# MiniMax-AI/VTP

Measured on NVIDIA H100. Metric: images/sec (256x256 encode+decode+3-loss step), higher is better.
Workload: dtype bf16

## Files before the change

vtp_b200/csrc/gemm.cu:

```cuda
#include <stdlib.h>

#include "host.h"
#include "ptx.cuh"

namespace vtp {

static constexpr int BM = 128;
static constexpr int BK = 64;
static constexpr int A_BYTES = BM * BK * 2;
static constexpr int NUM_THREADS = 512;
static constexpr int NUM_MMA_WARPS = 8;

struct GemmDev {
    int M, N, K;
    int a_mn, b_mn;
    int num_m_blocks, num_n_blocks, num_k_blocks, kb_per_split, num_splits;
    void* out;
    int ldo, out_dtype;
    const float* bias;
    int act, round_bf16;
    const void* resid;
    int ldr, resid_dtype;
    int accumulate;
    int rr_group, rr_skip;
    const __nv_bfloat16* rope_sin;
    const __nv_bfloat16* rope_cos;
    int rope_tokens, rope_prefix, rope_cols;
    int ps_r, ps_gh, ps_gw, ps_cout;
    __nv_bfloat16* out2;
    int ldo2;
    int conv_C, conv_H, conv_W, conv_TW, conv_TH, conv_tiles_h, conv_tiles_w, conv_B;
    const __nv_bfloat16* mask_pos;
    int ldm;
};
// ... 267 lines not shown
            store_half<PS>(p, stg, lane, grow0, orow8, ocol0, h, ncols, Nout, 0, has_resid);
            __syncwarp();
        }
    }
}


__device__ __forceinline__ int acc_key(int r) { return ((r & 3) << 1) | ((r >> 2) & 1); }

__device__ __forceinline__ void acc_ld32(const float* arow, int col0, int key, uint32_t (&r)[32]) {
#pragma unroll
    for (int i = 0; i < 8; ++i) {
        const float4 v = *reinterpret_cast<const float4*>(arow + col0 + 4 * (i ^ key));
        r[4 * i] = __float_as_uint(v.x), r[4 * i + 1] = __float_as_uint(v.y), r[4 * i + 2] = __float_as_uint(v.z),
        r[4 * i + 3] = __float_as_uint(v.w);
    }
}

struct AccHandoff {
    uint64_t* full;
    uint64_t* empty;
    uint32_t phase;
    __device__ __forceinline__ void wait_full() const { mbar_wait(full, phase); }
    __device__ __forceinline__ void release(int lane) const {
        __syncwarp();
        if (lane == 0) mbar_arrive(empty);
    }
};

struct TileIter {
    int n, m, ks;
    int dn, dm, dks;
    int nn, nm;
    __device__ __forceinline__ TileIter(int t0, int stride, int num_n, int num_m) : nn(num_n), nm(num_m) {
        n = t0 % num_n;
        const int r = t0 / num_n;
        m = r % num_m, ks = r / num_m;
        dn = stride % num_n;
        const int rs = stride / num_n;
        dm = rs % num_m, dks = rs / num_m;
    }
    __device__ __forceinline__ void next() {
        n += dn, m += dm, ks += dks;
        if (n >= nn) n -= nn, ++m;
        if (m >= nm) m -= nm, ++ks;
    }
};

template <int BN, int FAST>
__device__ __forceinline__ void fast_swiglu_tile(const GemmDev& p, const CUtensorMap* tmO, const CUtensorMap* tmO2, uint8_t* stg,
                                                 uint8_t* stg2, float* bias_s, int lane, int q, const AccHandoff& ah,
                                                 const float* arow, int key, int m_blk, int n0) {
    static_assert(BN == 128, "one packed chunk pair = one 64-column hidden line per tile row");
    constexpr bool PRE = FAST == 6;
    const int m0 = m_blk * BM;
    const int N = p.N;
    ah.wait_full();
    {
#pragma unroll
        for (int j = 0; j < 2; ++j) {
            const int col0 = n0 + j * 64;
            const bool valid = col0 < N;
            uint32_t r0[32], r1[32];
            if (valid) {
                acc_ld32(arow, j * 64, key, r0);
                acc_ld32(arow, j * 64 + 32, key, r1);
            }
            if (j == 1) ah.release(lane);
            bias_s[lane] = (p.bias && col0 + lane < N) ? __ldg(p.bias + col0 + lane) : 0.f;
            bias_s[32 + lane] = (p.bias && col0 + 32 + lane < N) ? __ldg(p.bias + col0 + 32 + lane) : 0.f;
            if (lane == 0) bulk_wait_read0();
            __syncwarp();
            uint32_t hw[16];
            uint32_t xs[32];
// ... 26 lines not shown
#pragma unroll
            for (int c = 0; c < 4; ++c)
                *reinterpret_cast<uint4*>(stg2 + stgb_off(lane, 4 * j + c)) = make_uint4(hw[4 * c], hw[4 * c + 1], hw[4 * c + 2], hw[4 * c + 3]);
            if (PRE && valid) {
                fence_proxy_async_smem();
                __syncwarp();
                if (lane == 0) {
                    tma_store_2d(tmO2, stg, col0, m0 + q * 32);
                    bulk_commit();
                }
            }
        }
        fence_proxy_async_smem();
        __syncwarp();
        if (lane == 0) {
            tma_store_2d(tmO, stg2, n0 >> 1, m0 + q * 32);
            bulk_commit();
        }
    }
}

template <int BN, int ACT, int FAST>
__device__ __forceinline__ void fast_epilogue_tile(const GemmDev& p, const CUtensorMap* tmO, uint8_t* stg, float* bias_s,
                                                   int lane, int q, const AccHandoff& ah, const float* arow, int key,
                                                   int m_blk, int n0) {
    constexpr bool OF32 = FAST == 3 || FAST == 4;
    constexpr bool MASK = FAST == 5;
    constexpr bool RES = FAST == 2 || FAST == 4 || MASK;
    const int m0 = m_blk * BM;
    constexpr int CW = OF32 ? 32 : 64;
    constexpr int TCH = BN / CW;
    constexpr int PW = OF32 ? 4 : 8;
    const int N = p.N;
    long row = (long)m0 + q * 32 + lane;
    bool row_ok = row < p.M;
    int ctx = 0, cty = 0, cb = 0;
    if (p.conv_C) {
        ctx = m_blk % p.conv_tiles_w, cty = (m_blk / p.conv_tiles_w) % p.conv_tiles_h;
        cb = m_blk / (p.conv_tiles_w * p.conv_tiles_h);
        const int r = q * 32 + lane;
        const int h = cty * p.conv_TH + r / p.conv_TW, w = ctx * p.conv_TW + r % p.conv_TW;
        row = ((long)cb * p.conv_H + h) * p.conv_W + w;
        row_ok = h < p.conv_H && cb < p.conv_B;
    }
    const char* rrow = !RES ? nullptr
                       : MASK ? reinterpret_cast<const char*>(p.mask_pos) + row * (long)p.ldm * 2
                              : reinterpret_cast<const char*>(p.resid) + row * (long)p.ldr * (OF32 ? 4 : 2);

    float b0n = 0.f, b1n = 0.f;
    uint4 rr[8];
    auto load_bias = [&](int col0) {
        if (p.bias) {
            b0n = (col0 + lane < N) ? __ldg(p.bias + col0 + lane) : 0.f;
            if (!OF32) b1n = (col0 + 32 + lane < N) ? __ldg(p.bias + col0 + 32 + lane) : 0.f;
        }
    };
    auto load_resid = [&](int col0) {
#pragma unroll
        for (int i = 0; i < 8; ++i) {
            const int col = col0 + PW * i;
            rr[i] = (row_ok && col + PW <= N) ? *reinterpret_cast<const uint4*>(rrow + (long)col * (OF32 ? 4 : 2))
                                              : make_uint4(0, 0, 0, 0);
        }
    };
    load_bias(n0);
    if (RES) {
        load_resid(n0);
#pragma unroll
        for (int j = 1; j < TCH; ++j) {
            const int col = n0 + j * CW;
            if (row_ok && col < N) asm volatile("prefetch.global.L2 [%0];" ::"l"(rrow + (long)col * (OF32 ? 4 : 2)));
        }
    }
    ah.wait_full();
#pragma unroll
    for (int c = 0; c < TCH; ++c) {
        const int col0 = n0 + c * CW;
        if (col0 >= N) break;
        const bool last = (c == TCH - 1) || (col0 + CW >= N);
        const float b0 = b0n, b1 = b1n;
        if (!last) load_bias(col0 + CW);
        uint32_t r0[32], r1[32];
        acc_ld32(arow, c * CW, key, r0);
        if (!OF32) acc_ld32(arow, c * CW + 32, key, r1);
        if (last) ah.release(lane);
        bias_s[lane] = b0;
        if (!OF32) bias_s[32 + lane] = b1;
        if (lane == 0) bulk_wait_read0();
        __syncwarp();
        {
#pragma unroll
            for (int i = 0; i < 8; ++i) {
                if constexpr (OF32) {
                    const float4 b = *reinterpret_cast<const float4*>(bias_s + 4 * i);
                    float4 v = make_float4(__uint_as_float(r0[4 * i]) + b.x, __uint_as_float(r0[4 * i + 1]) + b.y,
                                           __uint_as_float(r0[4 * i + 2]) + b.z, __uint_as_float(r0[4 * i + 3]) + b.w);
                    if (p.round_bf16) v.x = bf16_round(v.x), v.y = bf16_round(v.y), v.z = bf16_round(v.z), v.w = bf16_round(v.w);
                    if (ACT == VTP_ACT_RELU) v.x = fmaxf(v.x, 0.f), v.y = fmaxf(v.y, 0.f), v.z = fmaxf(v.z, 0.f), v.w = fmaxf(v.w, 0.f);
                    if (RES)
                        v.x += __uint_as_float(rr[i].x), v.y += __uint_as_float(rr[i].y), v.z += __uint_as_float(rr[i].z),
                            v.w += __uint_as_float(rr[i].w);
                    *reinterpret_cast<float4*>(stg + stgb_off(lane, i)) = v;
                } else {
                    const float4 ba = *reinterpret_cast<const float4*>(bias_s + 8 * i);
                    const float4 bb = *reinterpret_cast<const float4*>(bias_s + 8 * i + 4);
                    const uint32_t* r = i < 4 ? r0 + 8 * i : r1 + 8 * (i - 4);
                    float v[8] = {__uint_as_float(r[0]) + ba.x, __uint_as_float(r[1]) + ba.y, __uint_as_float(r[2]) + ba.z,
                                  __uint_as_float(r[3]) + ba.w, __uint_as_float(r[4]) + bb.x, __uint_as_float(r[5]) + bb.y,
// ... 8 lines not shown
                    if (MASK) {
                        auto keep = [](uint32_t x, uint32_t mm) {
                            const uint32_t lo = ((mm & 0x7FFFu) != 0u && (mm & 0x8000u) == 0u) ? 0x0000FFFFu : 0u;
                            const uint32_t hi = ((mm & 0x7FFF0000u) != 0u && (mm & 0x80000000u) == 0u) ? 0xFFFF0000u : 0u;
                            return x & (lo | hi);
                        };
                        w.x = keep(w.x, rr[i].x), w.y = keep(w.y, rr[i].y), w.z = keep(w.z, rr[i].z), w.w = keep(w.w, rr[i].w);
                    } else if (RES) {
                        w.x = add_bf16x2(w.x, rr[i].x), w.y = add_bf16x2(w.y, rr[i].y), w.z = add_bf16x2(w.z, rr[i].z),
                        w.w = add_bf16x2(w.w, rr[i].w);
                    }
                    *reinterpret_cast<uint4*>(stg + stgb_off(lane, i)) = w;
                }
            }
            if (RES && !last) load_resid(col0 + CW);
            fence_proxy_async_smem();
            __syncwarp();
            if (lane == 0) {
                if (p.conv_C) tma_store_4d(tmO, stg, col0, ctx * p.conv_TW, cty * p.conv_TH + q * (32 / p.conv_TW), cb);
                else tma_store_2d(tmO, stg, col0, m0 + q * 32);
                bulk_commit();
            }
        }
    }
}

template <int BN, int STAGES, int TA, int TB>
__device__ __forceinline__ void gemm_mainloop(float (&acc)[BN / 2], uint8_t* ring, uint64_t* full_bar, uint64_t* empty_bar,
                                              int& s, uint32_t& ph, int nkb, int wg, int lane) {
    constexpr int STAGE_BYTES = A_BYTES + BN * BK * 2;
    int prev = -1;
    for (int kb = 0; kb < nkb; ++kb) {
        mbar_wait(&full_bar[s], ph);
        const uint32_t a_base = smem_u32(ring + s * STAGE_BYTES) + wg * 8192;
        const uint32_t b_base = smem_u32(ring + s * STAGE_BYTES + A_BYTES);
        wgmma_fence();
#pragma unroll
        for (int j = 0; j < BK / 16; ++j) {
            const uint64_t ad = TA ? wgmma_desc_sw128(a_base + j * 2048, 8192, 1024) : wgmma_desc_sw128(a_base + j * 32, 0, 1024);
            const uint64_t bd = TB ? wgmma_desc_sw128(b_base + j * 2048, 8192, 1024) : wgmma_desc_sw128(b_base + j * 32, 0, 1024);
            const uint32_t sc = (kb > 0 || j > 0) ? 1u : 0u;
            if constexpr (BN == 128) wgmma_m64n128_ss<TA, TB>(acc, ad, bd, sc);
            else wgmma_m64n64_ss<TA, TB>(acc, ad, bd, sc);
        }
        wgmma_commit();
        wgmma_wait<1>();
        fence_regs(acc);
        if (prev >= 0 && lane == 0) mbar_arrive(&empty_bar[prev]);
        prev = s;
        if (++s == STAGES) s = 0, ph ^= 1;
    }
    wgmma_wait<0>();
    fence_regs(acc);
    if (prev >= 0 && lane == 0) mbar_arrive(&empty_bar[prev]);
}

template <int BN, int STAGES, int ACT, bool PS, int FAST>
__global__ void __launch_bounds__(NUM_THREADS, 1)
gemm_kernel(const __grid_constant__ CUtensorMap tmA, const __grid_constant__ CUtensorMap tmB,
            const __grid_constant__ CUtensorMap tmO, const __grid_constant__ CUtensorMap tmO2, const GemmDev p) {
    static_assert(BN == 64 || BN == 128, "tile width");
    constexpr int B_BYTES = BN * BK * 2;
    constexpr int STAGE_BYTES = A_BYTES + B_BYTES;
    extern __shared__ __align__(1024) uint8_t smem_raw[];
    uint8_t* smem = reinterpret_cast<uint8_t*>((reinterpret_cast<uintptr_t>(smem_raw) + 1023) & ~uintptr_t(1023));
    constexpr int STG_BYTES = NUM_EPI_WARPS * STG_FLOATS * 4 * (FAST == 6 ? 2 : 1);
    uint8_t* ring = smem;
    float* acc_s = reinterpret_cast<float*>(ring + STAGES * STAGE_BYTES);
    float* stg_base = acc_s + BM * BN;
    float* bias_base = reinterpret_cast<float*>(reinterpret_cast<uint8_t*>(stg_base) + STG_BYTES);
    uint64_t* full_bar = reinterpret_cast<uint64_t*>(reinterpret_cast<uint8_t*>(bias_base) + (FAST ? NUM_EPI_WARPS * 256 : 0));
    uint64_t* empty_bar = full_bar + STAGES;
    uint64_t* acc_full = empty_bar + STAGES;
    uint64_t* acc_empty = acc_full + 1;

    const int warp = threadIdx.x >> 5;
    const int lane = threadIdx.x & 31;
    const int work_id = blockIdx.x;
    const int work_stride = gridDim.x;

    if (warp == 0 && lane == 0) {
        tma_prefetch_desc(&tmA);
        tma_prefetch_desc(&tmB);
        if (FAST) tma_prefetch_desc(&tmO);
        if (FAST == 6) tma_prefetch_desc(&tmO2);
        for (int s = 0; s < STAGES; ++s) mbar_init(&full_bar[s], 1), mbar_init(&empty_bar[s], NUM_MMA_WARPS);
        mbar_init(acc_full, NUM_MMA_WARPS);
        mbar_init(acc_empty, NUM_EPI_WARPS);
        fence_barrier_init();
    }
    __syncthreads();

    const int num_tiles = p.num_m_blocks * p.num_n_blocks * p.num_splits;
    if (warp < 4) {
        setmaxnreg_dec<40>();
        if (warp == 0 && lane == 0) {
            int s = 0;
            uint32_t ph = 0;
            TileIter ti(work_id, work_stride, p.num_n_blocks, p.num_m_blocks);
            for (int t = work_id; t < num_tiles; t += work_stride, ti.next()) {
                const int n_blk = ti.n, m_blk = ti.m, ks = ti.ks;
                const int kb0 = ks * p.kb_per_split;
                const int kb1 = min(kb0 + p.kb_per_split, p.num_k_blocks);
                const int m0 = m_blk * BM, n0 = n_blk * BN;
                int cv_x0 = 0, cv_y0 = 0, cv_b = 0, cv_c = 0, cv_dx = -1, cv_dy = -1;
                if (p.conv_C) {
                    cv_x0 = (m_blk % p.conv_tiles_w) * p.conv_TW;
                    cv_y0 = ((m_blk / p.conv_tiles_w) % p.conv_tiles_h) * p.conv_TH;
                    cv_b = m_blk / (p.conv_tiles_w * p.conv_tiles_h);
                    if (kb0 != 0) {
                        const int cpk = p.conv_C >> 6, tap = kb0 / cpk;
                        cv_c = (kb0 % cpk) << 6, cv_dx = tap % 3 - 1, cv_dy = tap / 3 - 1;
                    }
                }
                for (int kb = kb0; kb < kb1; ++kb) {
                    mbar_wait(&empty_bar[s], ph ^ 1);
                    uint8_t* sa = ring + s * STAGE_BYTES;
                    uint8_t* sb = sa + A_BYTES;
// ... 3 lines not shown
                        tma_load_4d(sa, &tmA, &full_bar[s], cv_c, cv_x0 + cv_dx, cv_y0 + cv_dy, cv_b);
                        cv_c += 64;
                        if (cv_c == p.conv_C) {
                            cv_c = 0;
                            if (++cv_dx == 2) cv_dx = -1, ++cv_dy;
                        }
                    } else if (!p.a_mn) {
                        tma_load_2d(sa, &tmA, &full_bar[s], k0, m0);
                    } else {
                        tma_load_2d(sa, &tmA, &full_bar[s], m0, k0);
                        tma_load_2d(sa + 8192, &tmA, &full_bar[s], m0 + 64, k0);
                    }
                    if (!p.b_mn) {
                        tma_load_2d(sb, &tmB, &full_bar[s], k0, n0);
                    } else {
#pragma unroll
                        for (int i = 0; i < BN / 64; ++i) tma_load_2d(sb + i * 8192, &tmB, &full_bar[s], n0 + 64 * i, k0);
                    }
                    if (++s == STAGES) s = 0, ph ^= 1;
                }
            }
        }
    } else if (warp < 4 + NUM_MMA_WARPS) {
        setmaxnreg_inc<144>();
        const int wg = (warp >> 2) - 1;
        const int tw = threadIdx.x & 127;
        int s = 0;
        uint32_t ph = 0, acc_ph = 0;
        TileIter ti(work_id, work_stride, p.num_n_blocks, p.num_m_blocks);
        for (int t = work_id; t < num_tiles; t += work_stride, ti.next()) {
            const int kb0 = ti.ks * p.kb_per_split;
            const int nkb = min(kb0 + p.kb_per_split, p.num_k_blocks) - kb0;
            float acc[BN / 2];
            if (p.a_mn) {
                if (p.b_mn) gemm_mainloop<BN, STAGES, 1, 1>(acc, ring, full_bar, empty_bar, s, ph, nkb, wg, lane);
                else gemm_mainloop<BN, STAGES, 1, 0>(acc, ring, full_bar, empty_bar, s, ph, nkb, wg, lane);
            } else {
                if (p.b_mn) gemm_mainloop<BN, STAGES, 0, 1>(acc, ring, full_bar, empty_bar, s, ph, nkb, wg, lane);
                else gemm_mainloop<BN, STAGES, 0, 0>(acc, ring, full_bar, empty_bar, s, ph, nkb, wg, lane);
            }
            mbar_wait(acc_empty, acc_ph ^ 1);
            {
                const int r0 = 64 * wg + 16 * (tw >> 5) + ((tw & 31) >> 2), c0 = 2 * (tw & 3);
                const int key = acc_key(r0);
#pragma unroll
                for (int j = 0; j < BN / 8; ++j) {
                    const int off = 4 * ((2 * j + (c0 >> 2)) ^ key) + (c0 & 3);
                    *reinterpret_cast<float2*>(acc_s + r0 * BN + off) = make_float2(acc[4 * j], acc[4 * j + 1]);
                    *reinterpret_cast<float2*>(acc_s + (r0 + 8) * BN + off) = make_float2(acc[4 * j + 2], acc[4 * j + 3]);
                }
            }
            __syncwarp();
            if (lane == 0) mbar_arrive(acc_full);
            acc_ph ^= 1;
        }
    } else {
        setmaxnreg_inc<184>();
        const int q = warp & 3;
        float* stg = stg_base + q * STG_FLOATS;
        const bool has_resid = p.resid != nullptr;
        const float* arow = acc_s + (q * 32 + lane) * BN;
        const int key = acc_key(lane);
        AccHandoff ah{acc_full, acc_empty, 0};
        TileIter ti(work_id, work_stride, p.num_n_blocks, p.num_m_blocks);
        for (int t = work_id; t < num_tiles; t += work_stride, ti.next(), ah.phase ^= 1) {
            const int m_blk = ti.m, n0 = ti.n * BN;
            const int m0 = m_blk * BM;
            const int grow0 = m0 + q * 32;
            if constexpr (FAST == 6 || FAST == 7) {
                uint8_t* st1 = reinterpret_cast<uint8_t*>(stg);
                uint8_t* st2 = FAST == 6 ? reinterpret_cast<uint8_t*>(stg_base) + (NUM_EPI_WARPS + q) * STG_FLOATS * 4 : st1;
                fast_swiglu_tile<BN, FAST>(p, &tmO, &tmO2, st1, st2, bias_base + q * 64, lane, q, ah, arow, key, m_blk, n0);
                continue;
            }
            if constexpr (FAST != 0) {
                fast_epilogue_tile<BN, ACT, FAST>(p, &tmO, reinterpret_cast<uint8_t*>(stg), bias_base + q * 64, lane, q, ah,
                                                  arow, key, m_blk, n0);
                continue;
            }
            constexpr bool sw = ACT == VTP_ACT_SWIGLU8;
            long orow8[8];
#pragma unroll
            for (int it = 0; it < 8; ++it) orow8[it] = out_row(p, grow0 + 4 * it + (lane >> 3));
            uint32_t hold[16];
            ah.wait_full();
#pragma unroll 1
            for (int u = 0; u < BN / 64; ++u) {
                const int col0 = n0 + u * 64;
                if (col0 >= p.N) break;
                if (has_resid)
                    prefetch_resid_l2(p, lane, orow8, sw ? col0 >> 1 : col0, sw ? 32 : 64, sw ? p.N >> 1 : p.N);
                uint32_t r0[32], r1[32];
                acc_ld32(arow, u * 64, key, r0);
                acc_ld32(arow, u * 64 + 32, key, r1);
                if (u == BN / 64 - 1 || col0 + 64 >= p.N) ah.release(lane);
                float v[64];
#pragma unroll
                for (int i = 0; i < 32; ++i) v[i] = __uint_as_float(r0[i]), v[32 + i] = __uint_as_float(r1[i]);
                epilogue_unit<ACT, PS>(p, stg, lane, v, grow0, orow8, col0, has_resid, sw ? (u & 1) : 0, hold);
            }
        }
        if (FAST && lane == 0) bulk_wait0();
    }
}

template <int BN, int STAGES, int ACT, bool PS, int FAST = 0>
static int launch_gemm(const CUtensorMap& tmA, const CUtensorMap& tmB, const GemmDev& p, cudaStream_t stream,
                       const CUtensorMap* tmO = nullptr, const CUtensorMap* tmO2 = nullptr) {
    constexpr int smem_bytes = 1024 + STAGES * (A_BYTES + BN * BK * 2) + BM * BN * 4 +
                               NUM_EPI_WARPS * STG_FLOATS * 4 * (FAST == 6 ? 2 : 1) + (FAST ? NUM_EPI_WARPS * 256 : 0) +
                               (2 * STAGES + 2) * 8;
    static_assert(smem_bytes <= 232448, "shared memory budget (227 KB per block)");
    static bool configured = false;
    if (!configured) {
        VTP_CUDA(cudaFuncSetAttribute(gemm_kernel<BN, STAGES, ACT, PS, FAST>, cudaFuncAttributeMaxDynamicSharedMemorySize,
                                      smem_bytes));
        configured = true;
    }
    const int work = p.num_m_blocks * p.num_n_blocks * p.num_splits;
    const int grid = work < num_sms() ? work : num_sms();
    gemm_kernel<BN, STAGES, ACT, PS, FAST><<<grid, NUM_THREADS, smem_bytes, stream>>>(tmA, tmB, tmO ? *tmO : tmA,
                                                                                     tmO2 ? *tmO2 : tmA, p);
    VTP_LAUNCH_CHECK();
    return VTP_OK;
}

}

using namespace vtp;

extern "C" int vtp_gemm_bf16(const vtp_gemm_args* a, vtp_stream_t stream_) {
    cudaStream_t stream = reinterpret_cast<cudaStream_t>(stream_);
    VTP_CHECK_ARG(a != nullptr, "gemm: null args");
    VTP_CHECK_ARG(a->M > 0 && a->N > 0 && a->K > 0, "gemm: bad shape M=%d N=%d K=%d", a->M, a->N, a->K);
    VTP_CHECK_ARG(a->A && a->B && a->out, "gemm: null pointer");
    VTP_CHECK_ARG(a->lda % 8 == 0 && a->ldb % 8 == 0, "gemm: lda/ldb must be multiples of 8 (16B TMA strides)");
    VTP_CHECK_ARG((reinterpret_cast<uintptr_t>(a->A) & 15) == 0 && (reinterpret_cast<uintptr_t>(a->B) & 15) == 0,
                  "gemm: A/B must be 16B aligned");
    VTP_CHECK_ARG((reinterpret_cast<uintptr_t>(a->out) & 15) == 0, "gemm: out must be 16B aligned");
    VTP_CHECK_ARG(a->N % 8 == 0, "gemm: N must be a multiple of 8");
    VTP_CHECK_ARG(a->out_dtype == VTP_F32 || a->out_dtype == VTP_BF16, "gemm: bad out dtype");
    VTP_CHECK_ARG(a->ldo % (a->out_dtype == VTP_F32 ? 4 : 8) == 0 || a->ps_r > 0, "gemm: ldo alignment");
    int split_k = a->split_k < 1 ? 1 : a->split_k;
    const bool auto_split = a->split_k < 0 && a->accumulate && a->out_dtype == VTP_F32 && a->act == VTP_ACT_NONE && !a->bias;
    VTP_CHECK_ARG(split_k == 1 || (a->accumulate && a->out_dtype == VTP_F32 && a->act == VTP_ACT_NONE && !a->bias),
                  "gemm: split_k needs accumulate=1, fp32 out, no bias/activation");
    VTP_CHECK_ARG(!a->accumulate || a->out_dtype == VTP_F32, "gemm: accumulate needs fp32 out");
    if (a->act == VTP_ACT_ROPE)
        VTP_CHECK_ARG(a->rope_sin && a->rope_cos && a->rope_tokens > 0 && a->rope_cols % 64 == 0, "gemm: bad rope args");
    if (a->act == VTP_ACT_SWIGLU8) VTP_CHECK_ARG(a->N % 16 == 0, "gemm: swiglu needs N %% 16 == 0");
    if (a->ps_r > 0)
        VTP_CHECK_ARG(a->ps_r % 4 == 0 && a->M % (a->ps_gh * a->ps_gw) == 0 && a->N == a->ps_cout * a->ps_r * a->ps_r,
                      "gemm: bad pixel-shuffle args");
    if (a->resid) VTP_CHECK_ARG(a->ldr % (a->resid_dtype == VTP_F32 ? 4 : 8) == 0, "gemm: ldr alignment");
    if (a->out2) VTP_CHECK_ARG(a->ldo2 % 8 == 0, "gemm: ldo2 alignment");

    const bool conv = a->conv_C > 0;
    if (conv) {
        VTP_CHECK_ARG(a->conv_C % 64 == 0 && a->conv_H > 0 && a->conv_W % 4 == 0 && !a->a_mn_major && a->K == 9 * a->conv_C &&
                          a->M % (a->conv_H * a->conv_W) == 0 && a->rr_group == 0 && a->ps_r == 0,
                      "gemm(conv): need C %% 64 == 0, W %% 4 == 0, K == 9*C, M == B*H*W");
    }
    if (a->mask_pos) VTP_CHECK_ARG(a->out_dtype == VTP_BF16 && a->ldm % 8 == 0, "gemm: mask_pos needs bf16 out");
    int BN = a->N <= 64 ? 64 : 128;
    const bool allow_fast = getenv("VTP_GEMM_NO_FAST") == nullptr;
    const bool fast_conv = conv && a->out_dtype == VTP_BF16 && !a->resid && getenv("VTP_GEMM_CONV_NO_FAST") == nullptr;
    const bool fast = allow_fast && (!conv || fast_conv) && a->rr_group == 0 && a->ps_r == 0 && !a->out2 &&
                      (!a->mask_pos || fast_conv) && !a->accumulate && split_k == 1 &&
                      (a->act == VTP_ACT_NONE || (a->act == VTP_ACT_RELU && !a->mask_pos)) &&
                      (!a->resid || a->resid_dtype == a->out_dtype);
    const bool fast_swiglu = allow_fast && getenv("VTP_GEMM_NO_FAST_SWIGLU") == nullptr && a->act == VTP_ACT_SWIGLU8 && !conv &&
                             a->out_dtype == VTP_BF16 && a->round_bf16 && !a->resid && !a->mask_pos && !a->accumulate &&
                             split_k == 1 && a->rr_group == 0 && a->ps_r == 0 && a->ldo % 8 == 0;
    if (a->act == VTP_ACT_SWIGLU8) BN = 128;
    if (auto_split) {
        const int grid = num_sms();
        const int tiles = ceil_div(a->M, BM) * ceil_div(a->N, BN);
        const int nkb = ceil_div(a->K, BK);
        double best = -1.0;
        for (int sp = 1; sp <= 64 && sp * 8 <= (nkb > 8 ? nkb : 8); ++sp) {
            const int kps = ceil_div(nkb, sp);
            const int real = ceil_div(nkb, kps);
            const long work = (long)tiles * real;
            if (sp > 1 && work > 3L * grid) break;
            const double eff = (double)work / ((double)ceil_div((int)work, grid) * grid);
            if (eff > best + 0.02) best = eff, split_k = sp;
        }
// ... 43 lines not shown
        if (rc) return rc;
    }
    {
        uint64_t dims[2], strides[1] = {(uint64_t)a->ldb * 2};
        uint32_t box[2];
        if (!p.b_mn) dims[0] = a->K, dims[1] = a->N, box[0] = 64, box[1] = (uint32_t)BN;
        else dims[0] = a->N, dims[1] = a->K, box[0] = 64, box[1] = 64;
        int rc = make_tmap_bf16(&tmB, a->B, 2, dims, strides, box);
        if (rc) return rc;
    }
    if (fast_swiglu) {
        CUtensorMap tmH, tmP;
        {
            uint64_t dims[2] = {(uint64_t)a->N / 2, (uint64_t)a->M}, strides[1] = {(uint64_t)a->ldo * 2};
            uint32_t box[2] = {64, 32};
            int rc = make_tmap(&tmH, a->out, VTP_BF16, 2, dims, strides, box);
            if (rc) return rc;
        }
        if (a->out2) {
            uint64_t dims[2] = {(uint64_t)a->N, (uint64_t)a->M}, strides[1] = {(uint64_t)a->ldo2 * 2};
            uint32_t box[2] = {64, 32};
            int rc = make_tmap(&tmP, a->out2, VTP_BF16, 2, dims, strides, box);
            if (rc) return rc;
            return launch_gemm<128, 4, VTP_ACT_SWIGLU8, false, 6>(tmA, tmB, p, stream, &tmH, &tmP);
        }
        return launch_gemm<128, 4, VTP_ACT_SWIGLU8, false, 7>(tmA, tmB, p, stream, &tmH);
    }
    if (fast) {
        CUtensorMap tmO;
        const int esz = a->out_dtype == VTP_F32 ? 4 : 2;
        int rc;
        if (conv) {
            uint64_t dims[4] = {(uint64_t)a->N, (uint64_t)p.conv_W, (uint64_t)p.conv_H, (uint64_t)p.conv_B};
            uint64_t strides[3] = {(uint64_t)a->ldo * 2, (uint64_t)p.conv_W * a->ldo * 2, (uint64_t)p.conv_H * p.conv_W * a->ldo * 2};
            uint32_t box[4] = {64, (uint32_t)p.conv_TW, (uint32_t)(32 / p.conv_TW), 1};
            rc = make_tmap(&tmO, a->out, VTP_BF16, 4, dims, strides, box);
        } else {
            uint64_t dims[2] = {(uint64_t)a->N, (uint64_t)a->M}, strides[1] = {(uint64_t)a->ldo * esz};
            uint32_t box[2] = {(uint32_t)(128 / esz), 32};
            rc = make_tmap(&tmO, a->out, a->out_dtype, 2, dims, strides, box);
        }
        if (rc) return rc;
        const int mode = a->mask_pos ? 5 : (a->out_dtype == VTP_F32 ? 3 : 1) + (a->resid ? 1 : 0);
#define VTP_FAST_CFG(ACT_, MODE_)                                                                                     \
    return BN == 64 ? launch_gemm<64, 4, ACT_, false, MODE_>(tmA, tmB, p, stream, &tmO)                              \
                    : launch_gemm<128, 4, ACT_, false, MODE_>(tmA, tmB, p, stream, &tmO)
        if (mode == 5) VTP_FAST_CFG(VTP_ACT_NONE, 5);
#define VTP_FAST_ACT(ACT_)                                 \
    do {                                                   \
        switch (mode) {                                    \
            case 1: VTP_FAST_CFG(ACT_, 1);                 \
            case 2: VTP_FAST_CFG(ACT_, 2);                 \
            case 3: VTP_FAST_CFG(ACT_, 3);                 \
            default: VTP_FAST_CFG(ACT_, 4);                \
        }                                                  \
    } while (0)
        if (a->act == VTP_ACT_RELU) VTP_FAST_ACT(VTP_ACT_RELU);
        VTP_FAST_ACT(VTP_ACT_NONE);
#undef VTP_FAST_ACT
#undef VTP_FAST_CFG
    }
#define VTP_LAUNCH(ACT_, PS_)                                                              \
    return BN == 64 ? launch_gemm<64, 4, ACT_, PS_>(tmA, tmB, p, stream)                  \
                    : launch_gemm<128, 4, ACT_, PS_>(tmA, tmB, p, stream)
    if (a->ps_r > 0) {
        VTP_CHECK_ARG(a->act == VTP_ACT_NONE, "gemm: pixel shuffle has no activation");
        VTP_LAUNCH(VTP_ACT_NONE, true);
    }
    switch (a->act) {
        case VTP_ACT_NONE: VTP_LAUNCH(VTP_ACT_NONE, false);
        case VTP_ACT_GELU: VTP_LAUNCH(VTP_ACT_GELU, false);
        case VTP_ACT_SWIGLU8: return launch_gemm<128, 4, VTP_ACT_SWIGLU8, false>(tmA, tmB, p, stream);
        case VTP_ACT_ROPE: VTP_LAUNCH(VTP_ACT_ROPE, false);
        case VTP_ACT_RELU: VTP_LAUNCH(VTP_ACT_RELU, false);
        default: VTP_FAIL(VTP_ERR_ARG, "gemm: unknown activation %d", a->act);
    }
#undef VTP_LAUNCH
}
```

vtp_b200/csrc/ptx.cuh:

```cuda
#pragma once
#include <cuda_runtime.h>
#include <cuda_bf16.h>
#include <cuda.h>
#include <stdint.h>

namespace vtp {

__device__ __forceinline__ uint32_t smem_u32(const void* p) {
    return static_cast<uint32_t>(__cvta_generic_to_shared(p));
}
__device__ __forceinline__ uint32_t lane_id() { return threadIdx.x & 31; }

__device__ __forceinline__ bool elect_one() {
    uint32_t pred;
    asm volatile(
        "{\n\t.reg .pred p;\n\t"
        "elect.sync _|p, 0xffffffff;\n\t"
        "selp.u32 %0, 1, 0, p;\n\t}\n"
        : "=r"(pred));
    return pred != 0;
}

__device__ __forceinline__ void mbar_init(uint64_t* bar, uint32_t count) {
    asm volatile("mbarrier.init.shared::cta.b64 [%0], %1;" ::"r"(smem_u32(bar)), "r"(count));
// ... 115 lines not shown
__device__ __forceinline__ void setmaxnreg_dec() { asm volatile("setmaxnreg.dec.sync.aligned.u32 %0;" ::"n"(R)); }

template <int TA, int TB>
__device__ __forceinline__ void wgmma_m64n64_ss(float (&d)[32], uint64_t da, uint64_t db, uint32_t scale_d) {
    asm volatile(
        "{\n\t.reg .pred p;\n\t"
        "setp.ne.b32 p, %34, 0;\n\t"
        "wgmma.mma_async.sync.aligned.m64n64k16.f32.bf16.bf16 "
        "{%0,%1,%2,%3,%4,%5,%6,%7,%8,%9,%10,%11,%12,%13,%14,%15,%16,%17,%18,%19,%20,%21,%22,%23,%24,%25,%26,%27,%28,%29,%30,%31}, %32, %33, p, 1, 1, %35, %36;\n\t}\n"
        : "+f"(d[0]), "+f"(d[1]), "+f"(d[2]), "+f"(d[3]), "+f"(d[4]), "+f"(d[5]), "+f"(d[6]), "+f"(d[7]), "+f"(d[8]), "+f"(d[9]), "+f"(d[10]), "+f"(d[11]), "+f"(d[12]), "+f"(d[13]), "+f"(d[14]), "+f"(d[15]), "+f"(d[16]), "+f"(d[17]), "+f"(d[18]), "+f"(d[19]), "+f"(d[20]), "+f"(d[21]), "+f"(d[22]), "+f"(d[23]), "+f"(d[24]), "+f"(d[25]), "+f"(d[26]), "+f"(d[27]), "+f"(d[28]), "+f"(d[29]), "+f"(d[30]), "+f"(d[31])
        : "l"(da), "l"(db), "r"(scale_d), "n"(TA), "n"(TB));
}
template <int TA, int TB>
__device__ __forceinline__ void wgmma_m64n128_ss(float (&d)[64], uint64_t da, uint64_t db, uint32_t scale_d) {
    asm volatile(
        "{\n\t.reg .pred p;\n\t"
        "setp.ne.b32 p, %66, 0;\n\t"
        "wgmma.mma_async.sync.aligned.m64n128k16.f32.bf16.bf16 "
        "{%0,%1,%2,%3,%4,%5,%6,%7,%8,%9,%10,%11,%12,%13,%14,%15,%16,%17,%18,%19,%20,%21,%22,%23,%24,%25,%26,%27,%28,%29,%30,%31,%32,%33,%34,%35,%36,%37,%38,%39,%40,%41,%42,%43,%44,%45,%46,%47,%48,%49,%50,%51,%52,%53,%54,%55,%56,%57,%58,%59,%60,%61,%62,%63}, %64, %65, p, 1, 1, %67, %68;\n\t}\n"
        : "+f"(d[0]), "+f"(d[1]), "+f"(d[2]), "+f"(d[3]), "+f"(d[4]), "+f"(d[5]), "+f"(d[6]), "+f"(d[7]), "+f"(d[8]), "+f"(d[9]), "+f"(d[10]), "+f"(d[11]), "+f"(d[12]), "+f"(d[13]), "+f"(d[14]), "+f"(d[15]), "+f"(d[16]), "+f"(d[17]), "+f"(d[18]), "+f"(d[19]), "+f"(d[20]), "+f"(d[21]), "+f"(d[22]), "+f"(d[23]), "+f"(d[24]), "+f"(d[25]), "+f"(d[26]), "+f"(d[27]), "+f"(d[28]), "+f"(d[29]), "+f"(d[30]), "+f"(d[31]), "+f"(d[32]), "+f"(d[33]), "+f"(d[34]), "+f"(d[35]), "+f"(d[36]), "+f"(d[37]), "+f"(d[38]), "+f"(d[39]), "+f"(d[40]), "+f"(d[41]), "+f"(d[42]), "+f"(d[43]), "+f"(d[44]), "+f"(d[45]), "+f"(d[46]), "+f"(d[47]), "+f"(d[48]), "+f"(d[49]), "+f"(d[50]), "+f"(d[51]), "+f"(d[52]), "+f"(d[53]), "+f"(d[54]), "+f"(d[55]), "+f"(d[56]), "+f"(d[57]), "+f"(d[58]), "+f"(d[59]), "+f"(d[60]), "+f"(d[61]), "+f"(d[62]), "+f"(d[63])
        : "l"(da), "l"(db), "r"(scale_d), "n"(TA), "n"(TB));
}
template <int TA, int TB>
__device__ __forceinline__ void wgmma_m64n256_ss(float (&d)[128], uint64_t da, uint64_t db, uint32_t scale_d) {
    asm volatile(
        "{\n\t.reg .pred p;\n\t"
        "setp.ne.b32 p, %130, 0;\n\t"
        "wgmma.mma_async.sync.aligned.m64n256k16.f32.bf16.bf16 "
        "{%0,%1,%2,%3,%4,%5,%6,%7,%8,%9,%10,%11,%12,%13,%14,%15,%16,%17,%18,%19,%20,%21,%22,%23,%24,%25,%26,%27,%28,%29,%30,%31,%32,%33,%34,%35,%36,%37,%38,%39,%40,%41,%42,%43,%44,%45,%46,%47,%48,%49,%50,%51,%52,%53,%54,%55,%56,%57,%58,%59,%60,%61,%62,%63,%64,%65,%66,%67,%68,%69,%70,%71,%72,%73,%74,%75,%76,%77,%78,%79,%80,%81,%82,%83,%84,%85,%86,%87,%88,%89,%90,%91,%92,%93,%94,%95,%96,%97,%98,%99,%100,%101,%102,%103,%104,%105,%106,%107,%108,%109,%110,%111,%112,%113,%114,%115,%116,%117,%118,%119,%120,%121,%122,%123,%124,%125,%126,%127}, %128, %129, p, 1, 1, %131, %132;\n\t}\n"
        : "+f"(d[0]), "+f"(d[1]), "+f"(d[2]), "+f"(d[3]), "+f"(d[4]), "+f"(d[5]), "+f"(d[6]), "+f"(d[7]), "+f"(d[8]), "+f"(d[9]), "+f"(d[10]), "+f"(d[11]), "+f"(d[12]), "+f"(d[13]), "+f"(d[14]), "+f"(d[15]), "+f"(d[16]), "+f"(d[17]), "+f"(d[18]), "+f"(d[19]), "+f"(d[20]), "+f"(d[21]), "+f"(d[22]), "+f"(d[23]), "+f"(d[24]), "+f"(d[25]), "+f"(d[26]), "+f"(d[27]), "+f"(d[28]), "+f"(d[29]), "+f"(d[30]), "+f"(d[31]), "+f"(d[32]), "+f"(d[33]), "+f"(d[34]), "+f"(d[35]), "+f"(d[36]), "+f"(d[37]), "+f"(d[38]), "+f"(d[39]), "+f"(d[40]), "+f"(d[41]), "+f"(d[42]), "+f"(d[43]), "+f"(d[44]), "+f"(d[45]), "+f"(d[46]), "+f"(d[47]), "+f"(d[48]), "+f"(d[49]), "+f"(d[50]), "+f"(d[51]), "+f"(d[52]), "+f"(d[53]), "+f"(d[54]), "+f"(d[55]), "+f"(d[56]), "+f"(d[57]), "+f"(d[58]), "+f"(d[59]), "+f"(d[60]), "+f"(d[61]), "+f"(d[62]), "+f"(d[63]), "+f"(d[64]), "+f"(d[65]), "+f"(d[66]), "+f"(d[67]), "+f"(d[68]), "+f"(d[69]), "+f"(d[70]), "+f"(d[71]), "+f"(d[72]), "+f"(d[73]), "+f"(d[74]), "+f"(d[75]), "+f"(d[76]), "+f"(d[77]), "+f"(d[78]), "+f"(d[79]), "+f"(d[80]), "+f"(d[81]), "+f"(d[82]), "+f"(d[83]), "+f"(d[84]), "+f"(d[85]), "+f"(d[86]), "+f"(d[87]), "+f"(d[88]), "+f"(d[89]), "+f"(d[90]), "+f"(d[91]), "+f"(d[92]), "+f"(d[93]), "+f"(d[94]), "+f"(d[95]), "+f"(d[96]), "+f"(d[97]), "+f"(d[98]), "+f"(d[99]), "+f"(d[100]), "+f"(d[101]), "+f"(d[102]), "+f"(d[103]), "+f"(d[104]), "+f"(d[105]), "+f"(d[106]), "+f"(d[107]), "+f"(d[108]), "+f"(d[109]), "+f"(d[110]), "+f"(d[111]), "+f"(d[112]), "+f"(d[113]), "+f"(d[114]), "+f"(d[115]), "+f"(d[116]), "+f"(d[117]), "+f"(d[118]), "+f"(d[119]), "+f"(d[120]), "+f"(d[121]), "+f"(d[122]), "+f"(d[123]), "+f"(d[124]), "+f"(d[125]), "+f"(d[126]), "+f"(d[127])
        : "l"(da), "l"(db), "r"(scale_d), "n"(TA), "n"(TB));
}
template <int TB>
__device__ __forceinline__ void wgmma_m64n64_rs(float (&d)[32], const uint32_t (&a)[4], uint64_t db, uint32_t scale_d) {
    asm volatile(
        "{\n\t.reg .pred p;\n\t"
        "setp.ne.b32 p, %37, 0;\n\t"
        "wgmma.mma_async.sync.aligned.m64n64k16.f32.bf16.bf16 "
        "{%0,%1,%2,%3,%4,%5,%6,%7,%8,%9,%10,%11,%12,%13,%14,%15,%16,%17,%18,%19,%20,%21,%22,%23,%24,%25,%26,%27,%28,%29,%30,%31}, {%32,%33,%34,%35}, %36, p, 1, 1, %38;\n\t}\n"
        : "+f"(d[0]), "+f"(d[1]), "+f"(d[2]), "+f"(d[3]), "+f"(d[4]), "+f"(d[5]), "+f"(d[6]), "+f"(d[7]), "+f"(d[8]), "+f"(d[9]), "+f"(d[10]), "+f"(d[11]), "+f"(d[12]), "+f"(d[13]), "+f"(d[14]), "+f"(d[15]), "+f"(d[16]), "+f"(d[17]), "+f"(d[18]), "+f"(d[19]), "+f"(d[20]), "+f"(d[21]), "+f"(d[22]), "+f"(d[23]), "+f"(d[24]), "+f"(d[25]), "+f"(d[26]), "+f"(d[27]), "+f"(d[28]), "+f"(d[29]), "+f"(d[30]), "+f"(d[31])
        : "r"(a[0]), "r"(a[1]), "r"(a[2]), "r"(a[3]), "l"(db), "r"(scale_d), "n"(TB));
}

__device__ __forceinline__ uint32_t pack_bf16x2(float lo, float hi) {
    __nv_bfloat162 v = __floats2bfloat162_rn(lo, hi);
    return *reinterpret_cast<uint32_t*>(&v);
// ... 18 lines not shown
```

Before: 697.6.

## Add opt-in 192-wide GEMM tiles with split accumulator handoff and deeper BN64 ring

```diff
diff --git a/vtp_b200/csrc/gemm.cu b/vtp_b200/csrc/gemm.cu
--- a/vtp_b200/csrc/gemm.cu
+++ b/vtp_b200/csrc/gemm.cu
@@ -1,4 +1,5 @@
 #include <stdlib.h>
+#include <string.h>
 
 #include "host.h"
 #include "ptx.cuh"
@@ -10,6 +11,19 @@
 static constexpr int A_BYTES = BM * BK * 2;
 static constexpr int NUM_THREADS = 512;
 static constexpr int NUM_MMA_WARPS = 8;
+template <int BN, bool SWIGLU>
+struct TileCfg {
+    static constexpr int ACC_W = (SWIGLU || BN == 128) ? 128 : 64;
+    static constexpr int PARTS = (BN + ACC_W - 1) / ACC_W;
+    static constexpr int STAGES = (BN == 64 && !SWIGLU) ? 7 : 4;
+};
+
+template <int BN, int FAST>
+struct RegSplit {
+    static constexpr int PROD = 40;
+    static constexpr int MMA = BN <= 128 ? 144 : (FAST ? 152 : 160);
+    static constexpr int EPI = 512 - PROD - 2 * MMA;
+};
 
 struct GemmDev {
     int M, N, K;
@@ -323,11 +337,18 @@
     uint64_t* empty;
     uint32_t phase;
     __device__ __forceinline__ void wait_full() const { mbar_wait(full, phase); }
-    __device__ __forceinline__ void release(int lane) const {
+    __device__ __forceinline__ void release(int lane) {
         __syncwarp();
         if (lane == 0) mbar_arrive(empty);
+        phase ^= 1;
     }
 };
+
+template <int BN, int ACC_W>
+__device__ __forceinline__ int tile_parts(int n0, int N) {
+    const int p = (N - n0 + ACC_W - 1) / ACC_W;
+    return p < (BN + ACC_W - 1) / ACC_W ? p : (BN + ACC_W - 1) / ACC_W;
+}
 
 struct TileIter {
     int n, m, ks;
@@ -350,7 +371,7 @@
 
 template <int BN, int FAST>
 __device__ __forceinline__ void fast_swiglu_tile(const GemmDev& p, const CUtensorMap* tmO, const CUtensorMap* tmO2, uint8_t* stg,
-                                                 uint8_t* stg2, float* bias_s, int lane, int q, const AccHandoff& ah,
+                                                 uint8_t* stg2, float* bias_s, int lane, int q, AccHandoff& ah,
                                                  const float* arow, int key, int m_blk, int n0) {
     static_assert(BN == 128, "one packed chunk pair = one 64-column hidden line per tile row");
     constexpr bool PRE = FAST == 6;
@@ -423,7 +444,7 @@
 
 template <int BN, int ACT, int FAST>
 __device__ __forceinline__ void fast_epilogue_tile(const GemmDev& p, const CUtensorMap* tmO, uint8_t* stg, float* bias_s,
-                                                   int lane, int q, const AccHandoff& ah, const float* arow, int key,
+                                                   int lane, int q, AccHandoff& ah, const float* arow, int key,
                                                    int m_blk, int n0) {
     constexpr bool OF32 = FAST == 3 || FAST == 4;
     constexpr bool MASK = FAST == 5;
@@ -431,6 +452,8 @@
     const int m0 = m_blk * BM;
     constexpr int CW = OF32 ? 32 : 64;
     constexpr int TCH = BN / CW;
+    constexpr int ACC_W = TileCfg<BN, false>::ACC_W;
+    constexpr int CPH = ACC_W / CW < TCH ? ACC_W / CW : TCH;
     constexpr int PW = OF32 ? 4 : 8;
     const int N = p.N;
     long row = (long)m0 + q * 32 + lane;
@@ -473,18 +496,13 @@
             if (row_ok && col < N) asm volatile("prefetch.global.L2 [%0];" ::"l"(rrow + (long)col * (OF32 ? 4 : 2)));
         }
     }
-    ah.wait_full();
-#pragma unroll
-    for (int c = 0; c < TCH; ++c) {
-        const int col0 = n0 + c * CW;
-        if (col0 >= N) break;
-        const bool last = (c == TCH - 1) || (col0 + CW >= N);
+    auto chunk = [&](int acol, int col0, bool last, bool release) {
         const float b0 = b0n, b1 = b1n;
         if (!last) load_bias(col0 + CW);
         uint32_t r0[32], r1[32];
-        acc_ld32(arow, c * CW, key, r0);
-        if (!OF32) acc_ld32(arow, c * CW + 32, key, r1);
-        if (last) ah.release(lane);
+        acc_ld32(arow, acol, key, r0);
+        if (!OF32) acc_ld32(arow, acol + 32, key, r1);
+        if (release) ah.release(lane);
         bias_s[lane] = b0;
         if (!OF32) bias_s[32 + lane] = b1;
         if (lane == 0) bulk_wait_read0();
@@ -539,6 +557,32 @@
                 bulk_commit();
             }
         }
+    };
+    ah.wait_full();
+    if constexpr (BN <= ACC_W) {
+#pragma unroll
+        for (int c = 0; c < TCH; ++c) {
+            const int col0 = n0 + c * CW;
+            if (col0 >= N) break;
+            const bool last = (c == TCH - 1) || (col0 + CW >= N);
+            chunk(c * CW, col0, last, last);
+        }
+    } else {
+#pragma unroll 1
+        for (int h = 0; h < TileCfg<BN, false>::PARTS; ++h) {
+            if (h > 0) {
+                if (n0 + h * ACC_W >= N) break;
+                ah.wait_full();
+            }
+#pragma unroll
+            for (int cc = 0; cc < CPH; ++cc) {
+                const int c = h * CPH + cc;
+                const int col0 = n0 + c * CW;
+                if (c >= TCH || col0 >= N) break;
+                const bool last = (c == TCH - 1) || (col0 + CW >= N);
+                chunk(cc * CW, col0, last, last || cc == CPH - 1);
+            }
+        }
     }
 }
 
@@ -557,7 +601,9 @@
             const uint64_t ad = TA ? wgmma_desc_sw128(a_base + j * 2048, 8192, 1024) : wgmma_desc_sw128(a_base + j * 32, 0, 1024);
             const uint64_t bd = TB ? wgmma_desc_sw128(b_base + j * 2048, 8192, 1024) : wgmma_desc_sw128(b_base + j * 32, 0, 1024);
             const uint32_t sc = (kb > 0 || j > 0) ? 1u : 0u;
-            if constexpr (BN == 128) wgmma_m64n128_ss<TA, TB>(acc, ad, bd, sc);
+            if constexpr (BN == 256) wgmma_m64n256_ss<TA, TB>(acc, ad, bd, sc);
+            else if constexpr (BN == 192) wgmma_m64n192_ss<TA, TB>(acc, ad, bd, sc);
+            else if constexpr (BN == 128) wgmma_m64n128_ss<TA, TB>(acc, ad, bd, sc);
             else wgmma_m64n64_ss<TA, TB>(acc, ad, bd, sc);
         }
         wgmma_commit();
@@ -576,7 +622,9 @@
 __global__ void __launch_bounds__(NUM_THREADS, 1)
 gemm_kernel(const __grid_constant__ CUtensorMap tmA, const __grid_constant__ CUtensorMap tmB,
             const __grid_constant__ CUtensorMap tmO, const __grid_constant__ CUtensorMap tmO2, const GemmDev p) {
-    static_assert(BN == 64 || BN == 128, "tile width");
+    static_assert(BN == 64 || BN == 128 || BN == 192 || BN == 256, "tile width");
+    static_assert(STAGES == TileCfg<BN, ACT == VTP_ACT_SWIGLU8>::STAGES, "ring depth");
+    constexpr int ACC_W = TileCfg<BN, ACT == VTP_ACT_SWIGLU8>::ACC_W;
     constexpr int B_BYTES = BN * BK * 2;
     constexpr int STAGE_BYTES = A_BYTES + B_BYTES;
     extern __shared__ __align__(1024) uint8_t smem_raw[];
@@ -584,7 +632,7 @@
     constexpr int STG_BYTES = NUM_EPI_WARPS * STG_FLOATS * 4 * (FAST == 6 ? 2 : 1);
     uint8_t* ring = smem;
     float* acc_s = reinterpret_cast<float*>(ring + STAGES * STAGE_BYTES);
-    float* stg_base = acc_s + BM * BN;
+    float* stg_base = acc_s + BM * ACC_W;
     float* bias_base = reinterpret_cast<float*>(reinterpret_cast<uint8_t*>(stg_base) + STG_BYTES);
     uint64_t* full_bar = reinterpret_cast<uint64_t*>(reinterpret_cast<uint8_t*>(bias_base) + (FAST ? NUM_EPI_WARPS * 256 : 0));
     uint64_t* empty_bar = full_bar + STAGES;
@@ -610,7 +658,7 @@
 
     const int num_tiles = p.num_m_blocks * p.num_n_blocks * p.num_splits;
     if (warp < 4) {
-        setmaxnreg_dec<40>();
+        setmaxnreg_dec<RegSplit<BN, FAST>::PROD>();
         if (warp == 0 && lane == 0) {
             int s = 0;
             uint32_t ph = 0;
@@ -660,7 +708,7 @@
             }
         }
     } else if (warp < 4 + NUM_MMA_WARPS) {
-        setmaxnreg_inc<144>();
+        setmaxnreg_inc<RegSplit<BN, FAST>::MMA>();
         const int wg = (warp >> 2) - 1;
         const int tw = threadIdx.x & 127;
         int s = 0;
@@ -677,31 +725,36 @@
                 if (p.b_mn) gemm_mainloop<BN, STAGES, 0, 1>(acc, ring, full_bar, empty_bar, s, ph, nkb, wg, lane);
                 else gemm_mainloop<BN, STAGES, 0, 0>(acc, ring, full_bar, empty_bar, s, ph, nkb, wg, lane);
             }
-            mbar_wait(acc_empty, acc_ph ^ 1);
-            {
-                const int r0 = 64 * wg + 16 * (tw >> 5) + ((tw & 31) >> 2), c0 = 2 * (tw & 3);
-                const int key = acc_key(r0);
-#pragma unroll
-                for (int j = 0; j < BN / 8; ++j) {
-                    const int off = 4 * ((2 * j + (c0 >> 2)) ^ key) + (c0 & 3);
-                    *reinterpret_cast<float2*>(acc_s + r0 * BN + off) = make_float2(acc[4 * j], acc[4 * j + 1]);
-                    *reinterpret_cast<float2*>(acc_s + (r0 + 8) * BN + off) = make_float2(acc[4 * j + 2], acc[4 * j + 3]);
+            const int nh = tile_parts<BN, ACC_W>(ti.n * BN, p.N);
+            const int r0 = 64 * wg + 16 * (tw >> 5) + ((tw & 31) >> 2), c0 = 2 * (tw & 3);
+            const int key = acc_key(r0);
+#pragma unroll
+            for (int h = 0; h < (BN + ACC_W - 1) / ACC_W; ++h) {
+                if (h < nh) {
+                    mbar_wait(acc_empty, acc_ph ^ 1);
+#pragma unroll
+                    for (int jj = 0; jj < ACC_W / 8 && h * (ACC_W / 8) + jj < BN / 8; ++jj) {
+                        const int j = h * (ACC_W / 8) + jj;
+                        const int off = 4 * ((2 * jj + (c0 >> 2)) ^ key) + (c0 & 3);
+                        *reinterpret_cast<float2*>(acc_s + r0 * ACC_W + off) = make_float2(acc[4 * j], acc[4 * j + 1]);
+                        *reinterpret_cast<float2*>(acc_s + (r0 + 8) * ACC_W + off) = make_float2(acc[4 * j + 2], acc[4 * j + 3]);
+                    }
+                    __syncwarp();
+                    if (lane == 0) mbar_arrive(acc_full);
+                    acc_ph ^= 1;
                 }
             }
-            __syncwarp();
-            if (lane == 0) mbar_arrive(acc_full);
-            acc_ph ^= 1;
         }
     } else {
-        setmaxnreg_inc<184>();
+        setmaxnreg_inc<RegSplit<BN, FAST>::EPI>();
         const int q = warp & 3;
         float* stg = stg_base + q * STG_FLOATS;
         const bool has_resid = p.resid != nullptr;
-        const float* arow = acc_s + (q * 32 + lane) * BN;
+        const float* arow = acc_s + (q * 32 + lane) * ACC_W;
         const int key = acc_key(lane);
         AccHandoff ah{acc_full, acc_empty, 0};
         TileIter ti(work_id, work_stride, p.num_n_blocks, p.num_m_blocks);
-        for (int t = work_id; t < num_tiles; t += work_stride, ti.next(), ah.phase ^= 1) {
+        for (int t = work_id; t < num_tiles; t += work_stride, ti.next()) {
             const int m_blk = ti.m, n0 = ti.n * BN;
             const int m0 = m_blk * BM;
             const int grow0 = m0 + q * 32;
@@ -721,17 +774,20 @@
 #pragma unroll
             for (int it = 0; it < 8; ++it) orow8[it] = out_row(p, grow0 + 4 * it + (lane >> 3));
             uint32_t hold[16];
-            ah.wait_full();
+            constexpr int UPH = ACC_W / 64;
+            if (BN <= ACC_W) ah.wait_full();
 #pragma unroll 1
             for (int u = 0; u < BN / 64; ++u) {
                 const int col0 = n0 + u * 64;
                 if (col0 >= p.N) break;
                 if (has_resid)
                     prefetch_resid_l2(p, lane, orow8, sw ? col0 >> 1 : col0, sw ? 32 : 64, sw ? p.N >> 1 : p.N);
+                if (BN > ACC_W && u % UPH == 0) ah.wait_full();
+                const int acol = BN > ACC_W ? (u % UPH) * 64 : u * 64;
                 uint32_t r0[32], r1[32];
-                acc_ld32(arow, u * 64, key, r0);
-                acc_ld32(arow, u * 64 + 32, key, r1);
-                if (u == BN / 64 - 1 || col0 + 64 >= p.N) ah.release(lane);
+                acc_ld32(arow, acol, key, r0);
+                acc_ld32(arow, acol + 32, key, r1);
+                if (u == BN / 64 - 1 || col0 + 64 >= p.N || (BN > ACC_W && u % UPH == UPH - 1)) ah.release(lane);
                 float v[64];
 #pragma unroll
                 for (int i = 0; i < 32; ++i) v[i] = __uint_as_float(r0[i]), v[32 + i] = __uint_as_float(r1[i]);
@@ -742,10 +798,11 @@
     }
 }
 
-template <int BN, int STAGES, int ACT, bool PS, int FAST = 0>
+template <int BN, int ACT, bool PS, int FAST = 0>
 static int launch_gemm(const CUtensorMap& tmA, const CUtensorMap& tmB, const GemmDev& p, cudaStream_t stream,
                        const CUtensorMap* tmO = nullptr, const CUtensorMap* tmO2 = nullptr) {
-    constexpr int smem_bytes = 1024 + STAGES * (A_BYTES + BN * BK * 2) + BM * BN * 4 +
+    constexpr int STAGES = TileCfg<BN, ACT == VTP_ACT_SWIGLU8>::STAGES;
+    constexpr int smem_bytes = 1024 + STAGES * (A_BYTES + BN * BK * 2) + BM * TileCfg<BN, ACT == VTP_ACT_SWIGLU8>::ACC_W * 4 +
                                NUM_EPI_WARPS * STG_FLOATS * 4 * (FAST == 6 ? 2 : 1) + (FAST ? NUM_EPI_WARPS * 256 : 0) +
                                (2 * STAGES + 2) * 8;
     static_assert(smem_bytes <= 232448, "shared memory budget (227 KB per block)");
@@ -761,6 +818,28 @@
                                                                                      tmO2 ? *tmO2 : tmA, p);
     VTP_LAUNCH_CHECK();
     return VTP_OK;
+}
+
+template <int ACT, bool PS, int FAST>
+static constexpr bool kWide = FAST != 0 ? ACT != VTP_ACT_SWIGLU8 : (!PS && ACT != VTP_ACT_ROPE && ACT != VTP_ACT_SWIGLU8);
+
+template <int ACT, bool PS, int FAST = 0>
+static int launch_gemm_bn(int BN, const CUtensorMap& tmA, const CUtensorMap& tmB, const GemmDev& p, cudaStream_t stream,
+                          const CUtensorMap* tmO = nullptr) {
+    if constexpr (kWide<ACT, PS, FAST>)
+        if (BN == 192) return launch_gemm<192, ACT, PS, FAST>(tmA, tmB, p, stream, tmO);
+    if (BN == 64) return launch_gemm<64, ACT, PS, FAST>(tmA, tmB, p, stream, tmO);
+    return launch_gemm<128, ACT, PS, FAST>(tmA, tmB, p, stream, tmO);
+}
+
+static int choose_bn(int N, bool wide_ok) {
+    const char* env = getenv("VTP_GEMM_BN");
+    if (env && *env && strcmp(env, "auto") != 0) {
+        const int f = atoi(env);
+        if (f == 64 || f == 128 || (f == 192 && wide_ok)) return f;
+        if (f == 192) return 128;
+    }
+    return N <= 64 ? 64 : 128;
 }
 
 }
@@ -800,7 +879,8 @@
                       "gemm(conv): need C %% 64 == 0, W %% 4 == 0, K == 9*C, M == B*H*W");
     }
     if (a->mask_pos) VTP_CHECK_ARG(a->out_dtype == VTP_BF16 && a->ldm % 8 == 0, "gemm: mask_pos needs bf16 out");
-    int BN = a->N <= 64 ? 64 : 128;
+    const bool wide_ok = a->act != VTP_ACT_SWIGLU8 && a->act != VTP_ACT_ROPE && a->ps_r == 0;
+    int BN = choose_bn(a->N, wide_ok);
     const bool allow_fast = getenv("VTP_GEMM_NO_FAST") == nullptr;
     const bool fast_conv = conv && a->out_dtype == VTP_BF16 && !a->resid && getenv("VTP_GEMM_CONV_NO_FAST") == nullptr;
     const bool fast = allow_fast && (!conv || fast_conv) && a->rr_group == 0 && a->ps_r == 0 && !a->out2 &&
@@ -890,9 +970,9 @@
             uint32_t box[2] = {64, 32};
             int rc = make_tmap(&tmP, a->out2, VTP_BF16, 2, dims, strides, box);
             if (rc) return rc;
-            return launch_gemm<128, 4, VTP_ACT_SWIGLU8, false, 6>(tmA, tmB, p, stream, &tmH, &tmP);
-        }
-        return launch_gemm<128, 4, VTP_ACT_SWIGLU8, false, 7>(tmA, tmB, p, stream, &tmH);
+            return launch_gemm<128, VTP_ACT_SWIGLU8, false, 6>(tmA, tmB, p, stream, &tmH, &tmP);
+        }
+        return launch_gemm<128, VTP_ACT_SWIGLU8, false, 7>(tmA, tmB, p, stream, &tmH);
     }
     if (fast) {
         CUtensorMap tmO;
@@ -910,9 +990,7 @@
         }
         if (rc) return rc;
         const int mode = a->mask_pos ? 5 : (a->out_dtype == VTP_F32 ? 3 : 1) + (a->resid ? 1 : 0);
-#define VTP_FAST_CFG(ACT_, MODE_)                                                                                     \
-    return BN == 64 ? launch_gemm<64, 4, ACT_, false, MODE_>(tmA, tmB, p, stream, &tmO)                              \
-                    : launch_gemm<128, 4, ACT_, false, MODE_>(tmA, tmB, p, stream, &tmO)
+#define VTP_FAST_CFG(ACT_, MODE_) return launch_gemm_bn<ACT_, false, MODE_>(BN, tmA, tmB, p, stream, &tmO)
         if (mode == 5) VTP_FAST_CFG(VTP_ACT_NONE, 5);
 #define VTP_FAST_ACT(ACT_)                                 \
     do {                                                   \
@@ -928,9 +1006,7 @@
 #undef VTP_FAST_ACT
 #undef VTP_FAST_CFG
     }
-#define VTP_LAUNCH(ACT_, PS_)                                                              \
-    return BN == 64 ? launch_gemm<64, 4, ACT_, PS_>(tmA, tmB, p, stream)                  \
-                    : launch_gemm<128, 4, ACT_, PS_>(tmA, tmB, p, stream)
+#define VTP_LAUNCH(ACT_, PS_) return launch_gemm_bn<ACT_, PS_>(BN, tmA, tmB, p, stream)
     if (a->ps_r > 0) {
         VTP_CHECK_ARG(a->act == VTP_ACT_NONE, "gemm: pixel shuffle has no activation");
         VTP_LAUNCH(VTP_ACT_NONE, true);
@@ -938,7 +1014,7 @@
     switch (a->act) {
         case VTP_ACT_NONE: VTP_LAUNCH(VTP_ACT_NONE, false);
         case VTP_ACT_GELU: VTP_LAUNCH(VTP_ACT_GELU, false);
-        case VTP_ACT_SWIGLU8: return launch_gemm<128, 4, VTP_ACT_SWIGLU8, false>(tmA, tmB, p, stream);
+        case VTP_ACT_SWIGLU8: return launch_gemm<128, VTP_ACT_SWIGLU8, false>(tmA, tmB, p, stream);
         case VTP_ACT_ROPE: VTP_LAUNCH(VTP_ACT_ROPE, false);
         case VTP_ACT_RELU: VTP_LAUNCH(VTP_ACT_RELU, false);
         default: VTP_FAIL(VTP_ERR_ARG, "gemm: unknown activation %d", a->act);
diff --git a/vtp_b200/csrc/ptx.cuh b/vtp_b200/csrc/ptx.cuh
--- a/vtp_b200/csrc/ptx.cuh
+++ b/vtp_b200/csrc/ptx.cuh
@@ -161,6 +161,16 @@
         : "l"(da), "l"(db), "r"(scale_d), "n"(TA), "n"(TB));
 }
 template <int TA, int TB>
+__device__ __forceinline__ void wgmma_m64n192_ss(float (&d)[96], uint64_t da, uint64_t db, uint32_t scale_d) {
+    asm volatile(
+        "{\n\t.reg .pred p;\n\t"
+        "setp.ne.b32 p, %98, 0;\n\t"
+        "wgmma.mma_async.sync.aligned.m64n192k16.f32.bf16.bf16 "
+        "{%0,%1,%2,%3,%4,%5,%6,%7,%8,%9,%10,%11,%12,%13,%14,%15,%16,%17,%18,%19,%20,%21,%22,%23,%24,%25,%26,%27,%28,%29,%30,%31,%32,%33,%34,%35,%36,%37,%38,%39,%40,%41,%42,%43,%44,%45,%46,%47,%48,%49,%50,%51,%52,%53,%54,%55,%56,%57,%58,%59,%60,%61,%62,%63,%64,%65,%66,%67,%68,%69,%70,%71,%72,%73,%74,%75,%76,%77,%78,%79,%80,%81,%82,%83,%84,%85,%86,%87,%88,%89,%90,%91,%92,%93,%94,%95}, %96, %97, p, 1, 1, %99, %100;\n\t}\n"
+        : "+f"(d[0]), "+f"(d[1]), "+f"(d[2]), "+f"(d[3]), "+f"(d[4]), "+f"(d[5]), "+f"(d[6]), "+f"(d[7]), "+f"(d[8]), "+f"(d[9]), "+f"(d[10]), "+f"(d[11]), "+f"(d[12]), "+f"(d[13]), "+f"(d[14]), "+f"(d[15]), "+f"(d[16]), "+f"(d[17]), "+f"(d[18]), "+f"(d[19]), "+f"(d[20]), "+f"(d[21]), "+f"(d[22]), "+f"(d[23]), "+f"(d[24]), "+f"(d[25]), "+f"(d[26]), "+f"(d[27]), "+f"(d[28]), "+f"(d[29]), "+f"(d[30]), "+f"(d[31]), "+f"(d[32]), "+f"(d[33]), "+f"(d[34]), "+f"(d[35]), "+f"(d[36]), "+f"(d[37]), "+f"(d[38]), "+f"(d[39]), "+f"(d[40]), "+f"(d[41]), "+f"(d[42]), "+f"(d[43]), "+f"(d[44]), "+f"(d[45]), "+f"(d[46]), "+f"(d[47]), "+f"(d[48]), "+f"(d[49]), "+f"(d[50]), "+f"(d[51]), "+f"(d[52]), "+f"(d[53]), "+f"(d[54]), "+f"(d[55]), "+f"(d[56]), "+f"(d[57]), "+f"(d[58]), "+f"(d[59]), "+f"(d[60]), "+f"(d[61]), "+f"(d[62]), "+f"(d[63]), "+f"(d[64]), "+f"(d[65]), "+f"(d[66]), "+f"(d[67]), "+f"(d[68]), "+f"(d[69]), "+f"(d[70]), "+f"(d[71]), "+f"(d[72]), "+f"(d[73]), "+f"(d[74]), "+f"(d[75]), "+f"(d[76]), "+f"(d[77]), "+f"(d[78]), "+f"(d[79]), "+f"(d[80]), "+f"(d[81]), "+f"(d[82]), "+f"(d[83]), "+f"(d[84]), "+f"(d[85]), "+f"(d[86]), "+f"(d[87]), "+f"(d[88]), "+f"(d[89]), "+f"(d[90]), "+f"(d[91]), "+f"(d[92]), "+f"(d[93]), "+f"(d[94]), "+f"(d[95])
+        : "l"(da), "l"(db), "r"(scale_d), "n"(TA), "n"(TB));
+}
+template <int TA, int TB>
 __device__ __forceinline__ void wgmma_m64n256_ss(float (&d)[128], uint64_t da, uint64_t db, uint32_t scale_d) {
     asm volatile(
         "{\n\t.reg .pred p;\n\t"
```

Measured after the change: 698.1, median of 6. About the same (+0.1%).
